# wfus/Fully-Homomorphic-Image-Processing

Measured on AMD Instinct MI355X. Metric: encrypted 8x8 blocks/sec (homomorphic DCT+quant), higher is better.
Workload: dtype f64

## Files before the change

### fully-homomorphic-image-processing_amd/csrc/dct_fused.hip

```cpp
#include "internal.h"

#include <cstdlib>

#include "fp64_core.h"

#pragma clang fp contract(off)

namespace {
using namespace fp64;

template <int L, int LE> struct Shape {
    static constexpr int N = 1 << L, E = 1 << LE, TP = N >> LE, NP = (L + LE - 1) / LE, LDS_WORDS = N + (N >> LE);
};
__host__ __device__ constexpr int g_lo(int L, int LE, int p) { return (L - LE * p - LE) < 0 ? 0 : (L - LE * p - LE); }
__host__ __device__ constexpr int g_stages(int L, int LE, int p) { return (L - LE * p) > LE ? LE : (L - LE * p); }
template <int LO, int LE> __device__ __forceinline__ int g_index(int tid, int r) {
    return ((tid >> LO) << (LO + LE)) | (r << LO) | (tid & ((1 << LO) - 1));
}
template <int LO, int LE> __device__ __forceinline__ int g_pad(int j) { return j + ((j >> (LO + LE)) << LO); }

template <int L, int LE, int P> struct PassTw {
    static constexpr int LO = g_lo(L, LE, P), S = g_stages(L, LE, P), NTW = (1 << LE) - 1;
    static constexpr int rb(int u) { return (L - 1 - (LE * P + u)) - LO; }
    static constexpr int count(int u) { return 1 << (LE - 1 - rb(u)); }
// ... 22 lines not shown
            double t[KB * M], wm[KB * M];
#pragma unroll
            for (int kb = 0; kb < KB; kb++) {
                const int b = b0 + kb, r0 = ((b >> rb) << (rb + 1)) | (b & ((1 << rb) - 1)), r1 = r0 | (1 << rb);
                const double wv = w[T::offset(u) + (r0 >> (rb + 1))];
#pragma unroll
                for (int m = 0; m < M; m++) { t[kb * M + m] = x[m][r1]; wm[kb * M + m] = wv; }
            }
            mmv<KB * M>(t, wm, p, pinv);
#pragma unroll
            for (int kb = 0; kb < KB; kb++) {
                const int b = b0 + kb, r0 = ((b >> rb) << (rb + 1)) | (b & ((1 << rb) - 1)), r1 = r0 | (1 << rb);
#pragma unroll
                for (int m = 0; m < M; m++) {
                    const double X = x[m][r0];
                    x[m][r0] = X + t[kb * M + m];
                    x[m][r1] = X - t[kb * M + m];
                }
            }
        }
    }
}

template <int L, int LE, int P, int M>
__device__ __forceinline__ void inv_pass(double (&x)[M][1 << LE], const double (&w)[(1 << LE) - 1], double ninv, double p, double pinv) {
    using T = PassTw<L, LE, P>;
    constexpr int E = 1 << LE, KB = (LE == 3) ? 2 : 1;
#pragma unroll
    for (int u = T::S - 1; u >= 0; u--) {
        const int sigma = LE * P + u, rb = T::rb(u);
        if (sigma == 0) {
#pragma unroll
            for (int b = 0; b < E / 2; b++) {
                const int r0 = ((b >> rb) << (rb + 1)) | (b & ((1 << rb) - 1)), r1 = r0 | (1 << rb);
                const double wv = w[T::offset(u) + (r0 >> (rb + 1))];
                double t[2 * M], wm[2 * M];
#pragma unroll
                for (int m = 0; m < M; m++) {
                    const double X = x[m][r0], Y = x[m][r1];
                    t[m] = X + Y; wm[m] = ninv;
                    t[M + m] = X - Y; wm[M + m] = wv;
                }
                mmv<2 * M>(t, wm, p, pinv);
#pragma unroll
                for (int m = 0; m < M; m++) { x[m][r0] = t[m]; x[m][r1] = t[M + m]; }
            }
        } else {
#pragma unroll
            for (int b0 = 0; b0 < E / 2; b0 += KB) {
                double t[KB * M], wm[KB * M];
#pragma unroll
                for (int kb = 0; kb < KB; kb++) {
                    const int b = b0 + kb, r0 = ((b >> rb) << (rb + 1)) | (b & ((1 << rb) - 1)), r1 = r0 | (1 << rb);
                    const double wv = w[T::offset(u) + (r0 >> (rb + 1))];
#pragma unroll
                    for (int m = 0; m < M; m++) {
                        const double X = x[m][r0], Y = x[m][r1];
                        x[m][r0] = X + Y;
                        t[kb * M + m] = X - Y; wm[kb * M + m] = wv;
                    }
                }
                mmv<KB * M>(t, wm, p, pinv);
#pragma unroll
                for (int kb = 0; kb < KB; kb++) {
                    const int b = b0 + kb, r0 = ((b >> rb) << (rb + 1)) | (b & ((1 << rb) - 1)), r1 = r0 | (1 << rb);
#pragma unroll
                    for (int m = 0; m < M; m++) x[m][r1] = t[kb * M + m];
                }
            }
        }
    }
}

template <int L, int LE, int LO_FROM, int LO_TO, int M>
__device__ __forceinline__ void transpose(double (&x)[M][1 << LE], double *lds, int tid, int &phase) {
    constexpr int PL = imin(LO_FROM, LO_TO), E = 1 << LE;
    constexpr bool WAVE_LOCAL = (Shape<L, LE>::TP <= 64) || (LO_FROM <= 6 && LO_TO <= 6);
#pragma unroll
    for (int m = 0; m < M; m++) {
        double *buf = lds + (phase & 1) * Shape<L, LE>::LDS_WORDS;
        phase++;
#pragma unroll
        for (int r = 0; r < E; r++) buf[g_pad<PL, LE>(g_index<LO_FROM, LE>(tid, r))] = x[m][r];
        if constexpr (WAVE_LOCAL) {
            __builtin_amdgcn_fence(__ATOMIC_RELEASE, "wavefront");
            __builtin_amdgcn_wave_barrier();
            __builtin_amdgcn_fence(__ATOMIC_ACQUIRE, "wavefront");
        } else {
            __syncthreads();
        }
#pragma unroll
        for (int r = 0; r < E; r++) x[m][r] = buf[g_pad<PL, LE>(g_index<LO_TO, LE>(tid, r))];
    }
}

template <int L, int LE, int M, typename PRE, int P = 0>
__device__ __forceinline__ void ntt_fwd(double (&x)[M][1 << LE], double (&w)[(1 << LE) - 1], const double *__restrict__ tw, double p, double pinv,
                                        double *lds, int tid, int &phase, PRE pre) {
    if constexpr (P + 1 < Shape<L, LE>::NP) {
        double wn[(1 << LE) - 1];
        if (LE >= 4) load_tw<L, LE, P + 1>(wn, tw, tid);
        fwd_pass<L, LE, P, M>(x, w, p, pinv);
        if (LE < 4) load_tw<L, LE, P + 1>(wn, tw, tid);
        if constexpr (P + 2 == Shape<L, LE>::NP) pre();
        transpose<L, LE, g_lo(L, LE, P), g_lo(L, LE, P + 1), M>(x, lds, tid, phase);
        ntt_fwd<L, LE, M, PRE, P + 1>(x, wn, tw, p, pinv, lds, tid, phase, pre);
    } else {
        fwd_pass<L, LE, P, M>(x, w, p, pinv);
    }
}
template <int L, int LE, int M, bool BIG, int P = Shape<L, LE>::NP - 1>
__device__ __forceinline__ void ntt_inv(double (&x)[M][1 << LE], double (&w)[(1 << LE) - 1], const double *__restrict__ itw, double p, double pinv,
                                        double *lds, int tid, int &phase) {
    if constexpr (P > 0) {
        double wn[(1 << LE) - 1];
        if (LE >= 4) load_tw<L, LE, P - 1>(wn, itw, tid);
        inv_pass<L, LE, P, M>(x, w, 0.0, p, pinv);
        if (LE < 4) load_tw<L, LE, P - 1>(wn, itw, tid);
        if constexpr (BIG) {
#pragma unroll
            for (int m = 0; m < M; m++)
#pragma unroll
                for (int r = 0; r < (1 << LE); r++) x[m][r] = red(x[m][r], p, pinv);
        }
        transpose<L, LE, g_lo(L, LE, P), g_lo(L, LE, P - 1), M>(x, lds, tid, phase);
        ntt_inv<L, LE, M, BIG, P - 1>(x, wn, itw, p, pinv, lds, tid, phase);
    } else {
        inv_pass<L, LE, P, M>(x, w, itw[0], p, pinv);
    }
}

constexpr double PACK_BIAS = 6755399441055744.0;
template <int E, int TP>
__device__ __forceinline__ void store_packed(char *__restrict__ ob, u32 vo, u32 so, const double (&x)[E]) {
    static_assert(E == 8, "packed layout is defined for 8 values per thread");
    u32 lo[8], hi[8];
#pragma unroll
    for (int r = 0; r < 8; r++) {
        const double t = x[r] + PACK_BIAS;
        lo[r] = (u32)__double2loint(t);
        hi[r] = (u32)__double2hiint(t);
    }
#pragma unroll
    for (int q = 0; q < 4; q++) *(u64 *)(ob + (size_t)(so + q * TP * 8) + vo) = (u64)lo[2 * q] | ((u64)lo[2 * q + 1] << 32);
    u32 h[2];
#pragma unroll
    for (int g = 0; g < 2; g++) {
        const u32 p01 = __builtin_amdgcn_perm(hi[4 * g + 1], hi[4 * g + 0], 0x0c0c0400u);
        const u32 p23 = __builtin_amdgcn_perm(hi[4 * g + 3], hi[4 * g + 2], 0x0c0c0400u);
        h[g] = __builtin_amdgcn_perm(p23, p01, 0x05040100u);
    }
// ... 113 lines not shown
        }
    }
}

__host__ __device__ constexpr int occ_waves(int tp, int lds_words) {
    return ((2 * lds_words * 16 <= 160 * 1024) ? 2 : 1) * tp / 256 < 1 ? 1 : ((2 * lds_words * 16 <= 160 * 1024) ? 2 : 1) * tp / 256;
}
template <int L, int LE> struct Occ { static constexpr int W = occ_waves(Shape<L, LE>::TP, Shape<L, LE>::LDS_WORDS); };

template <int L, int LE, bool BIG, bool PACK, bool LDSC>
__global__ __launch_bounds__((Shape<L, LE>::TP), (Occ<L, LE>::W)) void k_dct_rows(const u64 *__restrict__ in, double *__restrict__ mid,
                                                                  const double *__restrict__ consts, const double *__restrict__ tw_all,
                                                                  const Modulus *__restrict__ mods, u32 k) {
    __shared__ double lds[2 * Shape<L, LE>::LDS_WORDS];
    const Work wk = decode(blockIdx.x, k);
    const double p = (double)mods[wk.prime].q, pinv = 1.0 / p;
    const double *tw = tw_all + (size_t)wk.prime * Shape<L, LE>::N;
    if (wk.half) rows_body<L, LE, BIG, 1, PACK, LDSC>(in, mid, consts, tw, wk, p, pinv, k, lds);
    else rows_body<L, LE, BIG, 0, PACK, LDSC>(in, mid, consts, tw, wk, p, pinv, k, lds);
}

template <int L, int LE, bool BIG, int HALF, bool PACK>
__device__ __forceinline__ void cols_body(const double *__restrict__ mid, u64 *__restrict__ out, const double *__restrict__ consts,
                                          const double *__restrict__ itw, const Work &wk, double p, double pinv, u32 k, double *lds) {
    using SH = Shape<L, LE>;
    constexpr int N = SH::N, TP = SH::TP, E = SH::E, NC = HalfC<HALF>::NC, FIRST = HalfC<HALF>::FIRST;
    constexpr int LASTP = SH::NP - 1;
    const int tid = threadIdx.x;
    const size_t poly_words = (size_t)k * N, ct_words = 2 * poly_words;
    const size_t base = ((size_t)wk.blk * 64 + wk.line) * ct_words + (size_t)wk.poly * poly_words + (size_t)wk.prime * N;
    const size_t cstride = (size_t)k * N;
    const gwin_t win_mid = gwin(mid + base), win_out = gwin(out + base);
    const gwin_t win_c = gwin(consts + (size_t)FIRST * cstride + (size_t)wk.prime * N);
    const gwin_t win_s = gwin(consts + (size_t)(12 + 8 * HALF + wk.line) * cstride + (size_t)wk.prime * N);
    const u32 vo = (u32)tid * 8u, rsb = (u32)(ct_words * 64), csb = (u32)(cstride * 8);
    const double pbias = p + 4503599627370496.0;
    double cn[9], sn[4];
    auto fetch = [&](int r) {
#pragma unroll
        for (int i = 0; i < NC; i++) cn[i] = gld_f64(win_c, vo, (u32)i * csb + r * TP * 8);
#pragma unroll
        for (int m = 0; m < 4; m++) sn[m] = gld_f64(win_s, vo, (u32)(16 * m) * csb + r * TP * 8);
    };
    double wl[E - 1];
    if constexpr (!PACK) {
        fetch(0);
        load_tw<L, LE, LASTP>(wl, itw, tid);
    }
    double x[4][E];
    if constexpr (PACK) {
// ... 25 lines not shown
            for (int r = 0; r < E; r++) {
                const double A = gld_f64(win_mid, vo, (u32)m * rsb + r * TP * 8), B = gld_f64(win_mid, vo, (u32)(7 - m) * rsb + r * TP * 8);
                x[m][r] = HALF ? A - B : A + B;
            }
        }
    }
    if constexpr (PACK) load_tw<L, LE, LASTP>(wl, itw, tid);
#pragma unroll
    for (int r = 0; r < E; r++) {
        double c[9], sc[4];
        if (PACK) fetch(r);
#pragma unroll
        for (int i = 0; i < NC; i++) c[i] = cn[i];
#pragma unroll
        for (int m = 0; m < 4; m++) sc[m] = sn[m];
        if (!PACK && r + 1 < E) fetch(r + 1);
        line_half<HALF>(x[0][r], x[1][r], x[2][r], x[3][r], c, p, pinv);
        double y[4] = {x[0][r], x[1][r], x[2][r], x[3][r]};
        mmv<4>(y, sc, p, pinv);
#pragma unroll
        for (int m = 0; m < 4; m++) x[m][r] = y[m];
    }
    int phase = 0;
    ntt_inv<L, LE, 4, BIG>(x, wl, itw, p, pinv, lds, tid, phase);
#pragma unroll
    for (int m = 0; m < 4; m++) {
#pragma unroll
        for (int r = 0; r < E; r++) gst_u64(win_out, vo, (u32)(2 * m + HALF) * rsb + r * TP * 8, f64_to_residue(x[m][r], pbias));
    }
}

template <int L, int LE, bool BIG, bool PACK>
__global__ __launch_bounds__((Shape<L, LE>::TP), (Occ<L, LE>::W)) void k_dct_cols(const double *__restrict__ mid, u64 *__restrict__ out,
                                                                  const double *__restrict__ consts, const double *__restrict__ itw_all,
                                                                  const Modulus *__restrict__ mods, u32 k) {
    __shared__ double lds[2 * Shape<L, LE>::LDS_WORDS];
    const Work wk = decode(blockIdx.x, k);
    const double p = (double)mods[wk.prime].q, pinv = 1.0 / p;
    const double *itw = itw_all + (size_t)wk.prime * Shape<L, LE>::N;
    if (wk.half) cols_body<L, LE, BIG, 1, PACK>(mid, out, consts, itw, wk, p, pinv, k, lds);
    else cols_body<L, LE, BIG, 0, PACK>(mid, out, consts, itw, wk, p, pinv, k, lds);
}

template <int L, int LE>
__global__ __launch_bounds__((Shape<L, LE>::TP), (Occ<L, LE>::W)) void k_dct_one_launch(const u64 *__restrict__ in, double *__restrict__ mid, u64 *__restrict__ out,
                                                                        const double *__restrict__ consts, const double *__restrict__ tw_all,
                                                                        const double *__restrict__ itw_all, const Modulus *__restrict__ mods, u32 k,
                                                                        u32 n_blocks, u32 dist, u32 *__restrict__ arrived, u32 *__restrict__ err) {
    __shared__ double lds[2 * Shape<L, LE>::LDS_WORDS];
    const u32 xcd = blockIdx.x & 7, seq = blockIdx.x >> 3, chunk = seq >> 5, r = seq & 31;
    const bool is_row = r < 16;
    const long j = is_row ? (long)chunk : (long)chunk - (long)(dist & 0xffffu);
    const u32 n_units = n_blocks * 2 * k;
    if (j < 0) return;
    const u64 g = (u64)j * 8 + xcd;
    if (g >= n_units) return;
    Work wk;
    wk.prime = (u32)(g / (n_blocks * 2));
    const u32 rem = (u32)(g - (u64)wk.prime * n_blocks * 2);
    wk.blk = rem >> 1;
    wk.poly = rem & 1;
    wk.line = (r & 15) >> 1;
    wk.half = r & 1;
    const double p = (double)mods[wk.prime].q, pinv = 1.0 / p;
    if (is_row) {
        const double *tw = tw_all + (size_t)wk.prime * Shape<L, LE>::N;
        if (wk.half) rows_body<L, LE, false, 1, true, true>(in, mid, consts, tw, wk, p, pinv, k, lds);
        else rows_body<L, LE, false, 0, true, true>(in, mid, consts, tw, wk, p, pinv, k, lds);
        if (dist & 0x10000u) return;
        __syncthreads();
        if (threadIdx.x == 0) {
            __threadfence();
            atomicAdd(arrived + g, 1u);
        }
    } else {
        if (!(dist & 0x10000u) && threadIdx.x == 0) {
            u32 spins = 0;
            while (__hip_atomic_load(arrived + g, __ATOMIC_RELAXED, __HIP_MEMORY_SCOPE_AGENT) < 16u) {
                __builtin_amdgcn_s_sleep(8);
                if (++spins > (1u << 24)) { atomicExch(err, 1u); break; }
            }
            __threadfence();
        }
        __syncthreads();
        const double *itw = itw_all + (size_t)wk.prime * Shape<L, LE>::N;
        if (wk.half) cols_body<L, LE, false, 1, true>(mid, out, consts, itw, wk, p, pinv, k, lds);
        else cols_body<L, LE, false, 0, true>(mid, out, consts, itw, wk, p, pinv, k, lds);
    }
}

__global__ void k_consts_to_f64(const ulonglong2 *__restrict__ in, double *__restrict__ out, const Modulus *__restrict__ mods, u32 k, u32 n, u32 le, u32 total) {
    const u32 i = blockIdx.x * blockDim.x + threadIdx.x;
    if (i >= total) return;
    const u32 pos = i % n, rowbase = i - pos;
    const u32 tp = n >> le, r = pos / tp, t = pos % tp;
    const u32 j = (t << le) + r;
    const u32 src = (j & 15) * (n >> 4) + (j >> 4);
    const u64 q = mods[(i / n) % k].q;
    const u64 w = in[rowbase + src].x;
    out[i] = w > q / 2 ? -(double)(q - w) : (double)w;
}

template <int L, int LE>
__global__ __launch_bounds__((Shape<L, LE>::TP), (Occ<L, LE>::W)) void k_rgb2ycc_f64(u64 *__restrict__ R, u64 *__restrict__ G, u64 *__restrict__ Bc,
                                                                     const double *__restrict__ consts, const double *__restrict__ tw_all,
                                                                     const double *__restrict__ itw_all, const Modulus *__restrict__ mods,
                                                                     const u64 *__restrict__ yoff, u32 yoff_len, u32 k, u32 group, u64 gstride) {
    using SH = Shape<L, LE>;
    constexpr int N = SH::N, TP = SH::TP, E = SH::E, LASTP = SH::NP - 1;
    __shared__ double lds[2 * SH::LDS_WORDS];
    const int tid = threadIdx.x;
    const u32 per_prime = gridDim.x / k;
    const u32 prime = blockIdx.x / per_prime;
    const u32 pp = blockIdx.x - prime * per_prime;
    const u32 poly = pp & 1, pix = pp >> 1;
    const u64 q = mods[prime].q;
    const double p = (double)q, pinv = 1.0 / p;
    const double *tw = tw_all + (size_t)prime * N, *itw = itw_all + (size_t)prime * N;
    const size_t pix_off = group ? (size_t)(pix / group) * gstride + (size_t)(pix % group) * 2 * k * N : (size_t)pix * 2 * k * N;
    const size_t off = pix_off + ((size_t)poly * k + prime) * N + tid;
    double w0[E - 1];
    load_tw<L, LE, 0>(w0, tw, tid);
// ... 112 lines not shown
            dst[r * TP] = f64_to_u52(v);
        }
    }
}

}


static u32 dct_shape_le(const fhe_ctx *c) {
    if (c->opt.dct_le != 3) return 4;
    if (c->logn == 12 && c->max_prime_bits <= 40) return 3;
    if (c->logn == 13 || c->logn == 11) return 3;
    return 4;
}

bool fhe_dct_f64_supported(const fhe_ctx *c) {
    return c && c->qb.d_tw_f64 && c->max_prime_bits <= 47 && (c->logn >= 10 && c->logn <= 13);
}

int fhe_dct_f64_make_consts(const fhe_ctx *c, fhe_dct_plan *plan, hipStream_t st) {
    const u32 total = DCT_NCONST * c->k * c->n;
    HIP_TRY(hipMalloc(&plan->d_consts_f64, sizeof(double) * total));
    const u32 le = dct_shape_le(c);
    k_consts_to_f64<<<(total + 255) / 256, 256, 0, st>>>(plan->d_consts, plan->d_consts_f64, c->qb.d_mod, c->k, c->n, le, total);
    KERNEL_CHECK();
    return FHE_OK;
}



template <int L, int LE>
static void launch_pair(const fhe_ctx *c, const fhe_dct_plan *plan, const u64 *in, u64 *out, double *mid, unsigned grid, bool big, hipStream_t st, int which) {
    constexpr int TP = Shape<L, LE>::TP;
    if constexpr (LE == 4) {
        if (big) {
            if (which & 1) k_dct_rows<L, LE, true, false, false><<<grid, TP, 0, st>>>(in, mid, plan->d_consts_f64, c->qb.d_tw_f64, c->qb.d_mod, c->k);
            if (which & 2) k_dct_cols<L, LE, true, false><<<grid, TP, 0, st>>>(mid, out, plan->d_consts_f64, c->qb.d_itw_f64, c->qb.d_mod, c->k);
            return;
        }
    }
    if constexpr (LE == 3) {
        if (big) {
            if (which & 1) k_dct_rows<L, LE, true, false, false><<<grid, TP, 0, st>>>(in, mid, plan->d_consts_f64, c->qb.d_tw_f64, c->qb.d_mod, c->k);
            if (which & 2) k_dct_cols<L, LE, true, false><<<grid, TP, 0, st>>>(mid, out, plan->d_consts_f64, c->qb.d_itw_f64, c->qb.d_mod, c->k);
            return;
        }
        if (c->max_prime_bits <= 37 && c->opt.dct_pack) {
            if (which & 1) {
                if (c->opt.dct_ldsc) k_dct_rows<L, LE, false, true, true><<<grid, TP, 0, st>>>(in, mid, plan->d_consts_f64, c->qb.d_tw_f64, c->qb.d_mod, c->k);
                else k_dct_rows<L, LE, false, true, false><<<grid, TP, 0, st>>>(in, mid, plan->d_consts_f64, c->qb.d_tw_f64, c->qb.d_mod, c->k);
            }
            if (which & 2) k_dct_cols<L, LE, false, true><<<grid, TP, 0, st>>>(mid, out, plan->d_consts_f64, c->qb.d_itw_f64, c->qb.d_mod, c->k);
            return;
        }
    }
    {
        if (which & 1) k_dct_rows<L, LE, false, false, false><<<grid, TP, 0, st>>>(in, mid, plan->d_consts_f64, c->qb.d_tw_f64, c->qb.d_mod, c->k);
        if (which & 2) k_dct_cols<L, LE, false, false><<<grid, TP, 0, st>>>(mid, out, plan->d_consts_f64, c->qb.d_itw_f64, c->qb.d_mod, c->k);
    }
}

int fhe_dct_f64_launch(const fhe_ctx *c, const fhe_dct_plan *plan, const u64 *in, u64 *out, u64 n_blocks, double *mid, hipStream_t st, int which) {
    const u64 items = n_blocks * 8 * 2 * c->k;
    const u64 grid = items * 2;
    if (grid > 0x7fffffffULL) return fail(FHE_ERR_PARAM, "too many blocks for one launch");
    if ((u64)c->k * c->n >= (1ULL << 21)) return fail(FHE_ERR_PARAM, "fused FP64 path: a block of ciphertexts exceeds the 2 GiB addressing window");
    const bool big = c->max_prime_bits > 40;
    if (c->opt.dct_one_launch && which == 3 && c->logn == 12 && dct_shape_le(c) == 3 && c->max_prime_bits <= 37 && c->opt.dct_pack && c->d_arrived) {
        const u64 n_units = n_blocks * 2 * c->k;
        if (n_units > c->arrived_cap) return fail(FHE_ERR_PARAM, "one-launch experiment: wave too large for the arrival counters");
        HIP_TRY(hipMemsetAsync(c->d_arrived, 0, (n_units + 1) * sizeof(u32), st));
        const u32 dist = c->opt.dct_one_launch;
        const u64 chunks = (n_units + 7) / 8 + (dist & 0xffffu);
        k_dct_one_launch<12, 3><<<(unsigned)(chunks * 32 * 8), Shape<12, 3>::TP, 0, st>>>(in, mid, out, plan->d_consts_f64, c->qb.d_tw_f64, c->qb.d_itw_f64, c->qb.d_mod,
                                                                                       c->k, (u32)n_blocks, dist, c->d_arrived + 1, c->d_arrived);
        KERNEL_CHECK();
        u32 timed_out = 0;
        HIP_TRY(hipMemcpyAsync(&timed_out, c->d_arrived, sizeof(u32), hipMemcpyDeviceToHost, st));
        HIP_TRY(hipStreamSynchronize(st));
        if (timed_out) return fail(FHE_ERR_HIP, "one-launch experiment: a column workgroup timed out waiting for its row transforms; the output is incomplete");
        return FHE_OK;
    }
    switch (c->logn) {
        case 10: launch_pair<10, 4>(c, plan, in, out, mid, (unsigned)grid, big, st, which); break;
        case 11: launch_pair<11, 3>(c, plan, in, out, mid, (unsigned)grid, big, st, which); break;
        case 12: if (dct_shape_le(c) == 3) launch_pair<12, 3>(c, plan, in, out, mid, (unsigned)grid, false, st, which); else launch_pair<12, 4>(c, plan, in, out, mid, (unsigned)grid, big, st, which); break;
        case 13: if (dct_shape_le(c) == 3) launch_pair<13, 3>(c, plan, in, out, mid, (unsigned)grid, big, st, which); else launch_pair<13, 4>(c, plan, in, out, mid, (unsigned)grid, big, st, which); break;
        default: return fail(FHE_ERR_PARAM, "fused FP64 path supports n in {1024, 2048, 4096, 8192}");
    }
    KERNEL_CHECK();
    return FHE_OK;
}

bool fhe_rgb_f64_supported(const fhe_ctx *c) {
    return fhe_dct_f64_supported(c) && c->logn == 12 && c->max_prime_bits <= 40;
}

int fhe_rgb_f64_make_consts(const fhe_ctx *c, const ulonglong2 *d_c, double **out, hipStream_t st) {
    const u32 total = 9 * c->k * c->n;
    HIP_TRY(hipMalloc(out, sizeof(double) * total));
    k_consts_to_f64<<<(total + 255) / 256, 256, 0, st>>>(d_c, *out, c->qb.d_mod, c->k, c->n, 3, total);
    KERNEL_CHECK();
    return FHE_OK;
}

int fhe_rgb_f64_launch(const fhe_ctx *c, u64 *r, u64 *g, u64 *b, u64 count, const double *consts, const u64 *yoff, u32 yoff_len, hipStream_t st, u32 group, u64 gstride) {
    const u64 grid = count * 2 * c->k;
    if (grid > 0x7fffffffULL) return fail(FHE_ERR_PARAM, "too many pixels for one launch");
    k_rgb2ycc_f64<12, 3><<<(unsigned)grid, Shape<12, 3>::TP, 0, st>>>(r, g, b, consts, c->qb.d_tw_f64, c->qb.d_itw_f64, c->qb.d_mod, yoff, yoff_len, c->k, group, gstride);
    KERNEL_CHECK();
    return FHE_OK;
}

int fhe_poly_f64_launch(int mode, const fhe_ctx *c, const u64 *in, u64 *out, u64 n_polys, const ulonglong2 *plain, hipStream_t st) {
    const u64 grid2 = (n_polys / 2) * c->k, grid1 = n_polys * c->k;
    if (grid1 > 0x7fffffffULL) return fail(FHE_ERR_PARAM, "too many polynomials for one launch");
    constexpr int TP = Shape<12, 3>::TP;
#define LAUNCH_POLY(M, GRID)                                                                                                          \
    switch (mode) {                                                                                                                   \
        case 0: k_poly_f64<12, 3, M, 0><<<(unsigned)(GRID), TP, 0, st>>>(in, out, plain, c->qb.d_tw_f64, c->qb.d_itw_f64, c->qb.d_mod, c->k); break; \
        case 1: k_poly_f64<12, 3, M, 1><<<(unsigned)(GRID), TP, 0, st>>>(in, out, plain, c->qb.d_tw_f64, c->qb.d_itw_f64, c->qb.d_mod, c->k); break; \
        default: k_poly_f64<12, 3, M, 2><<<(unsigned)(GRID), TP, 0, st>>>(in, out, plain, c->qb.d_tw_f64, c->qb.d_itw_f64, c->qb.d_mod, c->k); break; \
    }
    if (n_polys % 2 == 0) { LAUNCH_POLY(2, grid2) } else { LAUNCH_POLY(1, grid1) }
// ... 135 lines not shown
__global__ __launch_bounds__((Shape<L, LE>::TP), (Occ<L, LE>::W)) void k_idct_cols(const double *__restrict__ mid, u64 *__restrict__ out,
                                                                   const double *__restrict__ consts, const double *__restrict__ itw_all,
                                                                   const Modulus *__restrict__ mods, u32 k) {
    __shared__ double lds[2 * Shape<L, LE>::LDS_WORDS];
    const Work wk = decode(blockIdx.x, k);
    const double p = (double)mods[wk.prime].q, pinv = 1.0 / p;
    const double *itw = itw_all + (size_t)wk.prime * Shape<L, LE>::N;
    if (wk.half) icols_body<L, LE, BIG, 1>(mid, out, consts, itw, wk, p, pinv, k, lds);
    else icols_body<L, LE, BIG, 0>(mid, out, consts, itw, wk, p, pinv, k, lds);
}

template <int L, int LE>
void launch_ipair(const fhe_ctx *c, const double *consts, const u64 *in, u64 *out, double *mid, unsigned grid, bool big, hipStream_t st) {
    constexpr int TP = Shape<L, LE>::TP;
    k_idct_rows<L, LE><<<grid, TP, 0, st>>>(in, mid, consts, c->qb.d_tw_f64, c->qb.d_mod, c->k);
    if (big) k_idct_cols<L, LE, true><<<grid, TP, 0, st>>>(mid, out, consts, c->qb.d_itw_f64, c->qb.d_mod, c->k);
    else k_idct_cols<L, LE, false><<<grid, TP, 0, st>>>(mid, out, consts, c->qb.d_itw_f64, c->qb.d_mod, c->k);
}
}

int fhe_idct_f64_make_consts(const fhe_ctx *c, const ulonglong2 *d_consts, double **out, hipStream_t st) {
    const u32 total = DCT_NCONST * c->k * c->n;
    HIP_TRY(hipMalloc(out, sizeof(double) * total));
    k_consts_to_f64<<<(total + 255) / 256, 256, 0, st>>>(d_consts, *out, c->qb.d_mod, c->k, c->n, dct_shape_le(c), total);
    KERNEL_CHECK();
    return FHE_OK;
}

int fhe_idct_f64_launch(const fhe_ctx *c, const double *consts, const u64 *in, u64 *out, u64 n_blocks, double *mid, hipStream_t st) {
    const u64 grid = n_blocks * 8 * 2 * c->k * 2;
    if (grid > 0x7fffffffULL) return fail(FHE_ERR_PARAM, "too many blocks for one launch");
    const bool big = c->max_prime_bits > 40;
    switch (c->logn) {
        case 10: launch_ipair<10, 4>(c, consts, in, out, mid, (unsigned)grid, big, st); break;
        case 11: launch_ipair<11, 3>(c, consts, in, out, mid, (unsigned)grid, big, st); break;
        case 12: if (dct_shape_le(c) == 3) launch_ipair<12, 3>(c, consts, in, out, mid, (unsigned)grid, big, st); else launch_ipair<12, 4>(c, consts, in, out, mid, (unsigned)grid, big, st); break;
        case 13: if (dct_shape_le(c) == 3) launch_ipair<13, 3>(c, consts, in, out, mid, (unsigned)grid, big, st); else launch_ipair<13, 4>(c, consts, in, out, mid, (unsigned)grid, big, st); break;
        default: return fail(FHE_ERR_PARAM, "fused FP64 path supports n in {1024, 2048, 4096, 8192}");
    }
    KERNEL_CHECK();
    return FHE_OK;
}
```

### fully-homomorphic-image-processing_amd/csrc/fhe_hip.hip

```cpp
#include "internal.h"

#include <cmath>
#include <cstdarg>
#include <cstdio>
#include <cstdlib>
#include <cstring>
#include <algorithm>
#include <condition_variable>
#include <mutex>
#include <string>
#include <vector>

#include "host_math.h"

static thread_local std::string g_err;
int fhe_fail(int code, const char *fmt, ...) {
    char buf[512];
    va_list ap;
    va_start(ap, fmt);
    vsnprintf(buf, sizeof buf, fmt, ap);
    va_end(ap);
    g_err = buf;
    return code;
}

extern "C" const char *fhe_last_error(void) { return g_err.c_str(); }
extern "C" uint32_t fhe_abi_version(void) { return FHE_ABI_VERSION; }

int fhe_build_base(BaseTables &B, const std::vector<u64> &primes, u32 n, u32 logn, bool want_f64) {
    using namespace hostmath;
    const size_t cnt = primes.size();
    B.primes = primes;
    std::vector<ulonglong2> tw(cnt * n), itw(cnt * n);
    B.h_mod.resize(cnt);
    for (size_t i = 0; i < cnt; ++i) {
        const u64 q = primes[i];
        const u64 psi = primitive_2n_root(q, n);
        if (!psi) return fail(FHE_ERR_PARAM, "no primitive 2n-th root modulo %llu", (unsigned long long)q);
        const u64 ipsi = invmod(psi, q), ninv = invmod(n % q, q);
        u64 p = 1, ip = 1;
        for (u32 j = 0; j < n; ++j) {
            const u32 r = bit_reverse(j, (int)logn);
            tw[i * n + r] = make_ulonglong2(p, shoup(p, q));
            itw[i * n + r] = make_ulonglong2(ip, shoup(ip, q));
            p = mulmod(p, psi, q);
            ip = mulmod(ip, ipsi, q);
        }
        itw[i * n + 0] = make_ulonglong2(ninv, shoup(ninv, q));
        const u64 w1 = mulmod(itw[i * n + 1].x, ninv, q);
        itw[i * n + 1] = make_ulonglong2(w1, shoup(w1, q));
        Modulus m;
        m.q = q;
        const int b = bit_length(q);
        m.mu = (u64)((((u128)1) << (2 * b)) / q);
        m.s1 = (u32)(b - 1);
        m.s2 = (u32)(b + 1);
        B.h_mod[i] = m;
    }
    HIP_TRY(hipMalloc(&B.d_tw, sizeof(ulonglong2) * cnt * n));
    HIP_TRY(hipMalloc(&B.d_itw, sizeof(ulonglong2) * cnt * n));
    HIP_TRY(hipMalloc(&B.d_mod, sizeof(Modulus) * cnt));
    HIP_TRY(hipMemcpy(B.d_tw, tw.data(), sizeof(ulonglong2) * cnt * n, hipMemcpyHostToDevice));
    HIP_TRY(hipMemcpy(B.d_itw, itw.data(), sizeof(ulonglong2) * cnt * n, hipMemcpyHostToDevice));
    HIP_TRY(hipMemcpy(B.d_mod, B.h_mod.data(), sizeof(Modulus) * cnt, hipMemcpyHostToDevice));
    bool a_all = true, b_all = true;
    std::vector<PmMod> pm(cnt);
    for (size_t i = 0; i < cnt; ++i) {
        const u64 q = primes[i];
        const int b = bit_length(q);
        if (b < 34 || b > 58) { a_all = b_all = false; break; }
        const u64 delta = (1ULL << b) - q;
// ... 30 lines not shown
            auto p3 = [logn](u32 idx) -> u32 {
                if (idx < 2) return idx;
                int sigma = 0;
                while ((2u << sigma) <= idx) sigma++;
                const int LE = 3, P = sigma / LE, lo = ((int)logn - LE * P - LE) < 0 ? 0 : ((int)logn - LE * P - LE), rb = ((int)logn - 1 - sigma) - lo;
                const u32 off = idx - (1u << sigma), cnt_i = 1u << (LE - 1 - rb), th = off / cnt_i, i = off % cnt_i;
                return (1u << sigma) + i * ((1u << sigma) / cnt_i) + th;
            };
            for (size_t i = 0; i < cnt; ++i) {
                const u64 q = primes[i];
                for (u32 j = 0; j < n; ++j) {
                    const u32 jp = p3(j);
                    twp[i * n + jp] = make_ulonglong2(tw[i * n + j].x, (u64)(((u128)tw[i * n + j].x << 31) % q));
                    itwp[i * n + jp] = make_ulonglong2(itw[i * n + j].x, (u64)(((u128)itw[i * n + j].x << 31) % q));
                }
            }
            HIP_TRY(hipMalloc(&B.d_tw_pm3, sizeof(ulonglong2) * cnt * n));
            HIP_TRY(hipMalloc(&B.d_itw_pm3, sizeof(ulonglong2) * cnt * n));
            HIP_TRY(hipMemcpy(B.d_tw_pm3, twp.data(), sizeof(ulonglong2) * cnt * n, hipMemcpyHostToDevice));
            HIP_TRY(hipMemcpy(B.d_itw_pm3, itwp.data(), sizeof(ulonglong2) * cnt * n, hipMemcpyHostToDevice));
        }
    }
    if (want_f64) {
        std::vector<double> twd(cnt * n), itwd(cnt * n);
        for (size_t i = 0; i < cnt; ++i) {
            const u64 q = primes[i];
            auto centred = [q](u64 w) { return w > q / 2 ? -(double)(q - w) : (double)w; };
            for (u32 j = 0; j < n; ++j) {
                twd[i * n + j] = centred(tw[i * n + j].x);
                itwd[i * n + j] = centred(itw[i * n + j].x);
            }
        }
        HIP_TRY(hipMalloc(&B.d_tw_f64, sizeof(double) * cnt * n));
        HIP_TRY(hipMalloc(&B.d_itw_f64, sizeof(double) * cnt * n));
        HIP_TRY(hipMemcpy(B.d_tw_f64, twd.data(), sizeof(double) * cnt * n, hipMemcpyHostToDevice));
        HIP_TRY(hipMemcpy(B.d_itw_f64, itwd.data(), sizeof(double) * cnt * n, hipMemcpyHostToDevice));
    }
    return FHE_OK;
}
void fhe_free_base(BaseTables &B) {
    if (B.d_tw) (void)hipFree(B.d_tw);
    if (B.d_itw) (void)hipFree(B.d_itw);
    if (B.d_mod) (void)hipFree(B.d_mod);
    if (B.d_tw_f64) (void)hipFree(B.d_tw_f64);
    if (B.d_itw_f64) (void)hipFree(B.d_itw_f64);
    if (B.d_tw_pm) (void)hipFree(B.d_tw_pm);
    if (B.d_itw_pm) (void)hipFree(B.d_itw_pm);
    if (B.d_pm) (void)hipFree(B.d_pm);
    if (B.d_tw_pm3) (void)hipFree(B.d_tw_pm3);
    if (B.d_itw_pm3) (void)hipFree(B.d_itw_pm3);
    B.d_tw_pm = B.d_itw_pm = B.d_tw_pm3 = B.d_itw_pm3 = nullptr;
    B.d_pm = nullptr;
    B.pm_class = 0;
    B.d_tw_f64 = B.d_itw_f64 = nullptr;
    B.d_tw = B.d_itw = nullptr;
    B.d_mod = nullptr;
}

static bool env_on(const char *name) { const char *e = getenv(name); return e && *e && !(e[0] == '0' && !e[1]); }

extern "C" int fhe_default_coeff_modulus(uint32_t n, int preset, uint64_t *q_out) {
    static const u64 s3_4096[] = {0xffffee001ULL, 0xffffc4001ULL, 0x1ffffe0001ULL};
    static const u64 s3_8192[] = {0x7fffffd8001ULL, 0x7fffffc8001ULL, 0xfffffffc001ULL, 0xffffff6c001ULL, 0xfffffebc001ULL};
    static const u64 s23_2048[] = {0x3fffffff000001ULL};
    static const u64 s23_4096[] = {0x7fffffff380001ULL, 0x3fffffff000001ULL};
    static const u64 s23_8192[] = {0x7fffffff380001ULL, 0x7ffffffef00001ULL, 0x3fffffff000001ULL, 0x3ffffffef40001ULL};
    static const u64 s23_16384[] = {0x7fffffff380001ULL, 0x7ffffffef00001ULL, 0x7ffffffeac0001ULL, 0x7ffffffe700001ULL, 0x7ffffffe600001ULL, 0x7ffffffe4c0001ULL,
                                    0x3fffffff000001ULL, 0x3ffffffef40001ULL};
    const u64 *src = nullptr;
    int cnt = 0;
#define PICK(a) do { src = a; cnt = (int)(sizeof(a) / sizeof(a[0])); } while (0)
    if (preset == 0) {
        if (n == 4096) PICK(s3_4096);
        else if (n == 8192) PICK(s3_8192);
        else if (n == 2048 || n == 1024) PICK(s23_2048);
        else if (n == 16384) PICK(s23_16384);
    } else if (preset == 1) {
        if (n == 2048 || n == 1024) PICK(s23_2048);
// ... 1533 lines not shown
```

### fully-homomorphic-image-processing_amd/csrc/fp64_core.h

```cpp
#pragma once
#include "internal.h"

#pragma clang fp contract(off)

namespace fp64 {

__device__ __forceinline__ double mm(double y, double w, double p, double pinv) {
    const double h = y * w;
    const double l = __builtin_fma(y, w, -h);
    const double q = __builtin_rint(h * pinv);
    return __builtin_fma(-q, p, h) + l;
}
__device__ __forceinline__ double red(double x, double p, double pinv) {
    return __builtin_fma(-__builtin_rint(x * pinv), p, x);
}
template <int K>
__device__ __forceinline__ void mmv(double (&y)[K], const double (&w)[K], double p, double pinv) {
    double h[K], l[K], q[K];
#pragma unroll
    for (int i = 0; i < K; i++) h[i] = y[i] * w[i];
#pragma unroll
    for (int i = 0; i < K; i++) q[i] = h[i] * pinv;
#pragma unroll
    for (int i = 0; i < K; i++) l[i] = __builtin_fma(y[i], w[i], -h[i]);
#pragma unroll
    for (int i = 0; i < K; i++) q[i] = __builtin_rint(q[i]);
#pragma unroll
    for (int i = 0; i < K; i++) h[i] = __builtin_fma(-q[i], p, h[i]);
#pragma unroll
    for (int i = 0; i < K; i++) y[i] = h[i] + l[i];
}

__device__ __forceinline__ double u52_to_f64(u64 v) { return __longlong_as_double((long long)(v | 0x4330000000000000ULL)) - 4503599627370496.0; }
__device__ __forceinline__ u64 f64_to_u52(double v) { return (u64)__double_as_longlong(v + 4503599627370496.0) & 0x000FFFFFFFFFFFFFULL; }
__device__ __forceinline__ double u52_biased(u64 v) { return __longlong_as_double((long long)(v | 0x4330000000000000ULL)); }
__device__ __forceinline__ u64 f64_to_residue(double v, double pbias) {
    return (u64)__double_as_longlong(v + (v < 0.0 ? pbias : 4503599627370496.0)) & 0x000FFFFFFFFFFFFFULL;
}

typedef u32 u32x2 __attribute__((ext_vector_type(2)));
typedef __amdgpu_buffer_rsrc_t gwin_t;
__device__ __forceinline__ gwin_t gwin(const void *base) {
    return __builtin_amdgcn_make_buffer_rsrc(const_cast<void *>(base), 0, -1, 0x00020000 );
}
__device__ __forceinline__ u64 gld_u64(gwin_t w, u32 voff, u32 soff) { return __builtin_bit_cast(u64, __builtin_amdgcn_raw_buffer_load_b64(w, voff, soff, 0)); }
__device__ __forceinline__ double gld_f64(gwin_t w, u32 voff, u32 soff) { return __builtin_bit_cast(double, __builtin_amdgcn_raw_buffer_load_b64(w, voff, soff, 0)); }
__device__ __forceinline__ void gst_u64(gwin_t w, u32 voff, u32 soff, u64 v) { __builtin_amdgcn_raw_buffer_store_b64(__builtin_bit_cast(u32x2, v), w, voff, soff, 0); }
__device__ __forceinline__ void gst_f64(gwin_t w, u32 voff, u32 soff, double v) { __builtin_amdgcn_raw_buffer_store_b64(__builtin_bit_cast(u32x2, v), w, voff, soff, 0); }

template <int HALF>
__device__ __forceinline__ void line_half(double &x0, double &x1, double &x2, double &x3, const double (&c)[9], double p, double pinv) {
    if constexpr (HALF == 0) {
        const double tmp10 = x0 + x3, tmp13 = x0 - x3, tmp11 = x1 + x2, tmp12 = x1 - x2;
        double y[3] = {tmp12 + tmp13, tmp13, tmp12};
        const double w[3] = {c[0], c[1], c[2]};
        mmv<3>(y, w, p, pinv);
        x0 = tmp10 + tmp11;
        x2 = tmp10 - tmp11;
        x1 = y[0] + y[1];
        x3 = y[0] + y[2];
// ... 35 lines not shown
```

### fully-homomorphic-image-processing_amd/csrc/internal.h

```cpp
#pragma once
#include "../../include/fhe_hip.h"

#include <hip/hip_runtime.h>

#include <mutex>
#include <string>
#include <vector>

#include "modarith.h"
#include "ntt_core.h"

int fhe_fail(int code, const char *fmt, ...) __attribute__((format(printf, 2, 3)));
#define fail fhe_fail
#define HIP_TRY(expr)                                                                             \
    do {                                                                                          \
        hipError_t e_ = (expr);                                                                   \
        if (e_ != hipSuccess) return fail(FHE_ERR_HIP, "%s: %s", #expr, hipGetErrorString(e_));   \
    } while (0)
#define KERNEL_CHECK()                                                                            \
    do {                                                                                          \
        hipError_t e_ = hipGetLastError();                                                        \
        if (e_ != hipSuccess) return fail(FHE_ERR_HIP, "kernel launch: %s", hipGetErrorString(e_)); \
    } while (0)

struct BaseTables {
    std::vector<u64> primes;
    ulonglong2 *d_tw = nullptr, *d_itw = nullptr;
    Modulus *d_mod = nullptr;
    std::vector<Modulus> h_mod;
    double *d_tw_f64 = nullptr, *d_itw_f64 = nullptr;
    ulonglong2 *d_tw_pm = nullptr, *d_itw_pm = nullptr;
    ulonglong2 *d_tw_pm3 = nullptr, *d_itw_pm3 = nullptr;
    PmMod *d_pm = nullptr;
    int pm_class = 0;
    RnsBase dev() const { return RnsBase{d_tw, d_itw, d_mod, (u32)primes.size(), d_tw_pm, d_itw_pm, d_pm}; }
};

struct FheOptions {
    bool force_u64 = false;
    bool dct_pipeline = false;
    u64 dct_wave_blocks = 256;
    int dct_le = 3;
    bool dct_pack = true;
    bool dct_ldsc = true;
    bool dct_u64_fused = true;
    u32 dct_one_launch = 0;
    bool ntt_nolazy = false;
    bool ntt_single = false;
    bool ntt_nopm = false;
    bool behz_aux61 = false;
    bool behz_chunk3 = false;
    bool behz_tensor_canon = false;
    bool behz_tensor_single = false;
// ... 115 lines not shown
```

Measured before the change: 87070.

## Fold inverse-NTT n^-1 scaling into DCT constants and skip final-stage sum reduction

The inverse NTT's final stage no longer multiplies the sum half by n^-1. That factor is instead pre-multiplied into the DCT column constants (consts index ≥ 12) when they are converted to f64, and the last stage uses the raw first twiddle from a new per-prime table. This removes a modular multiply per sum output in the last inverse butterfly stage. Where needed, the unreduced sums are reduced with a cheap floor-based residue at store time (packed, non-big path) or an explicit red. The change relies on bounds proven via static_assert and touches constant-generation layout, so correctness depends on the folded constants matching every consumer.

```diff
diff --git a/fully-homomorphic-image-processing_amd/csrc/dct_fused.hip b/fully-homomorphic-image-processing_amd/csrc/dct_fused.hip
--- a/fully-homomorphic-image-processing_amd/csrc/dct_fused.hip
+++ b/fully-homomorphic-image-processing_amd/csrc/dct_fused.hip
@@ -68,14 +68,14 @@
     }
 }
 
-template <int L, int LE, int P, int M>
-__device__ __forceinline__ void inv_pass(double (&x)[M][1 << LE], const double (&w)[(1 << LE) - 1], double ninv, double p, double pinv) {
+template <int L, int LE, int P, int M, bool NINV_FOLDED = false, bool RED_SUMS = false>
+__device__ __forceinline__ void inv_pass(double (&x)[M][1 << LE], const double (&w)[(1 << LE) - 1], double last, double p, double pinv) {
     using T = PassTw<L, LE, P>;
     constexpr int E = 1 << LE, KB = (LE == 3) ? 2 : 1;
 #pragma unroll
     for (int u = T::S - 1; u >= 0; u--) {
         const int sigma = LE * P + u, rb = T::rb(u);
-        if (sigma == 0) {
+        if (sigma == 0 && !NINV_FOLDED) {
 #pragma unroll
             for (int b = 0; b < E / 2; b++) {
                 const int r0 = ((b >> rb) << (rb + 1)) | (b & ((1 << rb) - 1)), r1 = r0 | (1 << rb);
@@ -84,7 +84,7 @@
 #pragma unroll
                 for (int m = 0; m < M; m++) {
                     const double X = x[m][r0], Y = x[m][r1];
-                    t[m] = X + Y; wm[m] = ninv;
+                    t[m] = X + Y; wm[m] = last;
                     t[M + m] = X - Y; wm[M + m] = wv;
                 }
                 mmv<2 * M>(t, wm, p, pinv);
@@ -98,7 +98,7 @@
 #pragma unroll
                 for (int kb = 0; kb < KB; kb++) {
                     const int b = b0 + kb, r0 = ((b >> rb) << (rb + 1)) | (b & ((1 << rb) - 1)), r1 = r0 | (1 << rb);
-                    const double wv = w[T::offset(u) + (r0 >> (rb + 1))];
+                    const double wv = (sigma == 0) ? last : w[T::offset(u) + (r0 >> (rb + 1))];
 #pragma unroll
                     for (int m = 0; m < M; m++) {
                         const double X = x[m][r0], Y = x[m][r1];
@@ -112,6 +112,10 @@
                     const int b = b0 + kb, r0 = ((b >> rb) << (rb + 1)) | (b & ((1 << rb) - 1)), r1 = r0 | (1 << rb);
 #pragma unroll
                     for (int m = 0; m < M; m++) x[m][r1] = t[kb * M + m];
+                    if (sigma == 0 && RED_SUMS) {
+#pragma unroll
+                        for (int m = 0; m < M; m++) x[m][r0] = red(x[m][r0], p, pinv);
+                    }
                 }
             }
         }
@@ -155,9 +159,9 @@
         fwd_pass<L, LE, P, M>(x, w, p, pinv);
     }
 }
-template <int L, int LE, int M, bool BIG, int P = Shape<L, LE>::NP - 1>
+template <int L, int LE, int M, bool BIG, bool NINV_FOLDED = false, bool RED_SUMS = false, int P = Shape<L, LE>::NP - 1>
 __device__ __forceinline__ void ntt_inv(double (&x)[M][1 << LE], double (&w)[(1 << LE) - 1], const double *__restrict__ itw, double p, double pinv,
-                                        double *lds, int tid, int &phase) {
+                                        double *lds, int tid, int &phase, double wlast = 0.0) {
     if constexpr (P > 0) {
         double wn[(1 << LE) - 1];
         if (LE >= 4) load_tw<L, LE, P - 1>(wn, itw, tid);
@@ -170,9 +174,10 @@
                 for (int r = 0; r < (1 << LE); r++) x[m][r] = red(x[m][r], p, pinv);
         }
         transpose<L, LE, g_lo(L, LE, P), g_lo(L, LE, P - 1), M>(x, lds, tid, phase);
-        ntt_inv<L, LE, M, BIG, P - 1>(x, wn, itw, p, pinv, lds, tid, phase);
+        ntt_inv<L, LE, M, BIG, NINV_FOLDED, RED_SUMS, P - 1>(x, wn, itw, p, pinv, lds, tid, phase, wlast);
     } else {
-        inv_pass<L, LE, P, M>(x, w, itw[0], p, pinv);
+        static_assert(PassTw<L, LE, 0>::rb(0) == LE - 1, "last inverse stage must pair slot r with slot r + E / 2");
+        inv_pass<L, LE, P, M, NINV_FOLDED, RED_SUMS>(x, w, NINV_FOLDED ? wlast : itw[0], p, pinv);
     }
 }
 
@@ -332,10 +337,13 @@
 
 template <int L, int LE, bool BIG, int HALF, bool PACK>
 __device__ __forceinline__ void cols_body(const double *__restrict__ mid, u64 *__restrict__ out, const double *__restrict__ consts,
-                                          const double *__restrict__ itw, const Work &wk, double p, double pinv, u32 k, double *lds) {
+                                          const double *__restrict__ itw, double wlast, const Work &wk, double p, double pinv, u32 k, double *lds) {
     using SH = Shape<L, LE>;
     constexpr int N = SH::N, TP = SH::TP, E = SH::E, NC = HalfC<HALF>::NC, FIRST = HalfC<HALF>::FIRST;
     constexpr int LASTP = SH::NP - 1;
+    constexpr bool FLOOR_RES = PACK && !BIG && L <= 13;
+    static_assert(!FLOOR_RES || (1 << L) * 6 / 10 < FLOOR_RESIDUE_MAX_RATIO, "sum outputs exceed the range f64_floor_residue is proven for");
+    constexpr bool RED_AT_STORE = !FLOOR_RES && L == 10, RED_IN_STAGE = !FLOOR_RES && !RED_AT_STORE;
     const int tid = threadIdx.x;
     const size_t poly_words = (size_t)k * N, ct_words = 2 * poly_words;
     const size_t base = ((size_t)wk.blk * 64 + wk.line) * ct_words + (size_t)wk.poly * poly_words + (size_t)wk.prime * N;
@@ -407,30 +415,37 @@
         for (int m = 0; m < 4; m++) x[m][r] = y[m];
     }
     int phase = 0;
-    ntt_inv<L, LE, 4, BIG>(x, wl, itw, p, pinv, lds, tid, phase);
+    ntt_inv<L, LE, 4, BIG, true, RED_IN_STAGE>(x, wl, itw, p, pinv, lds, tid, phase, wlast);
 #pragma unroll
     for (int m = 0; m < 4; m++) {
 #pragma unroll
-        for (int r = 0; r < E; r++) gst_u64(win_out, vo, (u32)(2 * m + HALF) * rsb + r * TP * 8, f64_to_residue(x[m][r], pbias));
+        for (int r = 0; r < E; r++) {
+            u64 o;
+            if (FLOOR_RES && r < E / 2) o = f64_floor_residue(x[m][r], p, pinv);
+            else if (RED_AT_STORE && r < E / 2) o = f64_to_residue(red(x[m][r], p, pinv), pbias);
+            else o = f64_to_residue(x[m][r], pbias);
+            gst_u64(win_out, vo, (u32)(2 * m + HALF) * rsb + r * TP * 8, o);
+        }
     }
 }
 
 template <int L, int LE, bool BIG, bool PACK>
 __global__ __launch_bounds__((Shape<L, LE>::TP), (Occ<L, LE>::W)) void k_dct_cols(const double *__restrict__ mid, u64 *__restrict__ out,
                                                                   const double *__restrict__ consts, const double *__restrict__ itw_all,
-                                                                  const Modulus *__restrict__ mods, u32 k) {
+                                                                  const double *__restrict__ itw1_all, const Modulus *__restrict__ mods, u32 k) {
     __shared__ double lds[2 * Shape<L, LE>::LDS_WORDS];
     const Work wk = decode(blockIdx.x, k);
     const double p = (double)mods[wk.prime].q, pinv = 1.0 / p;
     const double *itw = itw_all + (size_t)wk.prime * Shape<L, LE>::N;
-    if (wk.half) cols_body<L, LE, BIG, 1, PACK>(mid, out, consts, itw, wk, p, pinv, k, lds);
-    else cols_body<L, LE, BIG, 0, PACK>(mid, out, consts, itw, wk, p, pinv, k, lds);
+    const double wlast = itw1_all[wk.prime];
+    if (wk.half) cols_body<L, LE, BIG, 1, PACK>(mid, out, consts, itw, wlast, wk, p, pinv, k, lds);
+    else cols_body<L, LE, BIG, 0, PACK>(mid, out, consts, itw, wlast, wk, p, pinv, k, lds);
 }
 
 template <int L, int LE>
 __global__ __launch_bounds__((Shape<L, LE>::TP), (Occ<L, LE>::W)) void k_dct_one_launch(const u64 *__restrict__ in, double *__restrict__ mid, u64 *__restrict__ out,
                                                                         const double *__restrict__ consts, const double *__restrict__ tw_all,
-                                                                        const double *__restrict__ itw_all, const Modulus *__restrict__ mods, u32 k,
+                                                                        const double *__restrict__ itw_all, const double *__restrict__ itw1_all, const Modulus *__restrict__ mods, u32 k,
                                                                         u32 n_blocks, u32 dist, u32 *__restrict__ arrived, u32 *__restrict__ err) {
     __shared__ double lds[2 * Shape<L, LE>::LDS_WORDS];
     const u32 xcd = blockIdx.x & 7, seq = blockIdx.x >> 3, chunk = seq >> 5, r = seq & 31;
@@ -469,20 +484,27 @@
         }
         __syncthreads();
         const double *itw = itw_all + (size_t)wk.prime * Shape<L, LE>::N;
-        if (wk.half) cols_body<L, LE, false, 1, true>(mid, out, consts, itw, wk, p, pinv, k, lds);
-        else cols_body<L, LE, false, 0, true>(mid, out, consts, itw, wk, p, pinv, k, lds);
-    }
-}
-
-__global__ void k_consts_to_f64(const ulonglong2 *__restrict__ in, double *__restrict__ out, const Modulus *__restrict__ mods, u32 k, u32 n, u32 le, u32 total) {
+        const double wlast = itw1_all[wk.prime];
+        if (wk.half) cols_body<L, LE, false, 1, true>(mid, out, consts, itw, wlast, wk, p, pinv, k, lds);
+        else cols_body<L, LE, false, 0, true>(mid, out, consts, itw, wlast, wk, p, pinv, k, lds);
+    }
+}
+
+__global__ void k_consts_to_f64(const ulonglong2 *__restrict__ in, double *__restrict__ out, const Modulus *__restrict__ mods, u32 k, u32 n, u32 le, u32 total,
+                                const ulonglong2 *__restrict__ itw, u32 fold_first) {
     const u32 i = blockIdx.x * blockDim.x + threadIdx.x;
     if (i >= total) return;
     const u32 pos = i % n, rowbase = i - pos;
     const u32 tp = n >> le, r = pos / tp, t = pos % tp;
     const u32 j = (t << le) + r;
     const u32 src = (j & 15) * (n >> 4) + (j >> 4);
-    const u64 q = mods[(i / n) % k].q;
-    const u64 w = in[rowbase + src].x;
+    const u32 prime = (i / n) % k;
+    const u64 q = mods[prime].q;
+    u64 w = in[rowbase + src].x;
+    if (i / (k * n) >= fold_first) {
+        const ulonglong2 ninv = itw[(size_t)prime * n];
+        w = mul_shoup(w, ninv.x, ninv.y, q);
+    }
     out[i] = w > q / 2 ? -(double)(q - w) : (double)w;
 }
 
@@ -641,7 +663,7 @@
     const u32 total = DCT_NCONST * c->k * c->n;
     HIP_TRY(hipMalloc(&plan->d_consts_f64, sizeof(double) * total));
     const u32 le = dct_shape_le(c);
-    k_consts_to_f64<<<(total + 255) / 256, 256, 0, st>>>(plan->d_consts, plan->d_consts_f64, c->qb.d_mod, c->k, c->n, le, total);
+    k_consts_to_f64<<<(total + 255) / 256, 256, 0, st>>>(plan->d_consts, plan->d_consts_f64, c->qb.d_mod, c->k, c->n, le, total, c->qb.d_itw, 12);
     KERNEL_CHECK();
     return FHE_OK;
 }
@@ -654,14 +676,14 @@
     if constexpr (LE == 4) {
         if (big) {
             if (which & 1) k_dct_rows<L, LE, true, false, false><<<grid, TP, 0, st>>>(in, mid, plan->d_consts_f64, c->qb.d_tw_f64, c->qb.d_mod, c->k);
-            if (which & 2) k_dct_cols<L, LE, true, false><<<grid, TP, 0, st>>>(mid, out, plan->d_consts_f64, c->qb.d_itw_f64, c->qb.d_mod, c->k);
+            if (which & 2) k_dct_cols<L, LE, true, false><<<grid, TP, 0, st>>>(mid, out, plan->d_consts_f64, c->qb.d_itw_f64, c->qb.d_itw1_f64, c->qb.d_mod, c->k);
             return;
         }
     }
     if constexpr (LE == 3) {
         if (big) {
             if (which & 1) k_dct_rows<L, LE, true, false, false><<<grid, TP, 0, st>>>(in, mid, plan->d_consts_f64, c->qb.d_tw_f64, c->qb.d_mod, c->k);
-            if (which & 2) k_dct_cols<L, LE, true, false><<<grid, TP, 0, st>>>(mid, out, plan->d_consts_f64, c->qb.d_itw_f64, c->qb.d_mod, c->k);
+            if (which & 2) k_dct_cols<L, LE, true, false><<<grid, TP, 0, st>>>(mid, out, plan->d_consts_f64, c->qb.d_itw_f64, c->qb.d_itw1_f64, c->qb.d_mod, c->k);
             return;
         }
         if (c->max_prime_bits <= 37 && c->opt.dct_pack) {
@@ -669,13 +691,13 @@
                 if (c->opt.dct_ldsc) k_dct_rows<L, LE, false, true, true><<<grid, TP, 0, st>>>(in, mid, plan->d_consts_f64, c->qb.d_tw_f64, c->qb.d_mod, c->k);
                 else k_dct_rows<L, LE, false, true, false><<<grid, TP, 0, st>>>(in, mid, plan->d_consts_f64, c->qb.d_tw_f64, c->qb.d_mod, c->k);
             }
-            if (which & 2) k_dct_cols<L, LE, false, true><<<grid, TP, 0, st>>>(mid, out, plan->d_consts_f64, c->qb.d_itw_f64, c->qb.d_mod, c->k);
+            if (which & 2) k_dct_cols<L, LE, false, true><<<grid, TP, 0, st>>>(mid, out, plan->d_consts_f64, c->qb.d_itw_f64, c->qb.d_itw1_f64, c->qb.d_mod, c->k);
             return;
         }
     }
     {
         if (which & 1) k_dct_rows<L, LE, false, false, false><<<grid, TP, 0, st>>>(in, mid, plan->d_consts_f64, c->qb.d_tw_f64, c->qb.d_mod, c->k);
-        if (which & 2) k_dct_cols<L, LE, false, false><<<grid, TP, 0, st>>>(mid, out, plan->d_consts_f64, c->qb.d_itw_f64, c->qb.d_mod, c->k);
+        if (which & 2) k_dct_cols<L, LE, false, false><<<grid, TP, 0, st>>>(mid, out, plan->d_consts_f64, c->qb.d_itw_f64, c->qb.d_itw1_f64, c->qb.d_mod, c->k);
     }
 }
 
@@ -691,7 +713,7 @@
         HIP_TRY(hipMemsetAsync(c->d_arrived, 0, (n_units + 1) * sizeof(u32), st));
         const u32 dist = c->opt.dct_one_launch;
         const u64 chunks = (n_units + 7) / 8 + (dist & 0xffffu);
-        k_dct_one_launch<12, 3><<<(unsigned)(chunks * 32 * 8), Shape<12, 3>::TP, 0, st>>>(in, mid, out, plan->d_consts_f64, c->qb.d_tw_f64, c->qb.d_itw_f64, c->qb.d_mod,
+        k_dct_one_launch<12, 3><<<(unsigned)(chunks * 32 * 8), Shape<12, 3>::TP, 0, st>>>(in, mid, out, plan->d_consts_f64, c->qb.d_tw_f64, c->qb.d_itw_f64, c->qb.d_itw1_f64, c->qb.d_mod,
                                                                                        c->k, (u32)n_blocks, dist, c->d_arrived + 1, c->d_arrived);
         KERNEL_CHECK();
         u32 timed_out = 0;
@@ -718,7 +740,7 @@
 int fhe_rgb_f64_make_consts(const fhe_ctx *c, const ulonglong2 *d_c, double **out, hipStream_t st) {
     const u32 total = 9 * c->k * c->n;
     HIP_TRY(hipMalloc(out, sizeof(double) * total));
-    k_consts_to_f64<<<(total + 255) / 256, 256, 0, st>>>(d_c, *out, c->qb.d_mod, c->k, c->n, 3, total);
+    k_consts_to_f64<<<(total + 255) / 256, 256, 0, st>>>(d_c, *out, c->qb.d_mod, c->k, c->n, 3, total, c->qb.d_itw, ~0u);
     KERNEL_CHECK();
     return FHE_OK;
 }
@@ -900,7 +922,7 @@
 int fhe_idct_f64_make_consts(const fhe_ctx *c, const ulonglong2 *d_consts, double **out, hipStream_t st) {
     const u32 total = DCT_NCONST * c->k * c->n;
     HIP_TRY(hipMalloc(out, sizeof(double) * total));
-    k_consts_to_f64<<<(total + 255) / 256, 256, 0, st>>>(d_consts, *out, c->qb.d_mod, c->k, c->n, dct_shape_le(c), total);
+    k_consts_to_f64<<<(total + 255) / 256, 256, 0, st>>>(d_consts, *out, c->qb.d_mod, c->k, c->n, dct_shape_le(c), total, c->qb.d_itw, ~0u);
     KERNEL_CHECK();
     return FHE_OK;
 }
diff --git a/fully-homomorphic-image-processing_amd/csrc/fhe_hip.hip b/fully-homomorphic-image-processing_amd/csrc/fhe_hip.hip
--- a/fully-homomorphic-image-processing_amd/csrc/fhe_hip.hip
+++ b/fully-homomorphic-image-processing_amd/csrc/fhe_hip.hip
@@ -32,6 +32,7 @@
     const size_t cnt = primes.size();
     B.primes = primes;
     std::vector<ulonglong2> tw(cnt * n), itw(cnt * n);
+    std::vector<u64> itw1_plain(cnt);
     B.h_mod.resize(cnt);
     for (size_t i = 0; i < cnt; ++i) {
         const u64 q = primes[i];
@@ -47,6 +48,7 @@
             ip = mulmod(ip, ipsi, q);
         }
         itw[i * n + 0] = make_ulonglong2(ninv, shoup(ninv, q));
+        itw1_plain[i] = itw[i * n + 1].x;
         const u64 w1 = mulmod(itw[i * n + 1].x, ninv, q);
         itw[i * n + 1] = make_ulonglong2(w1, shoup(w1, q));
         Modulus m;
@@ -123,7 +125,7 @@
         }
     }
     if (want_f64) {
-        std::vector<double> twd(cnt * n), itwd(cnt * n);
+        std::vector<double> twd(cnt * n), itwd(cnt * n), itw1d(cnt);
         for (size_t i = 0; i < cnt; ++i) {
             const u64 q = primes[i];
             auto centred = [q](u64 w) { return w > q / 2 ? -(double)(q - w) : (double)w; };
@@ -131,11 +133,14 @@
                 twd[i * n + j] = centred(tw[i * n + j].x);
                 itwd[i * n + j] = centred(itw[i * n + j].x);
             }
+            itw1d[i] = centred(itw1_plain[i]);
         }
         HIP_TRY(hipMalloc(&B.d_tw_f64, sizeof(double) * cnt * n));
         HIP_TRY(hipMalloc(&B.d_itw_f64, sizeof(double) * cnt * n));
+        HIP_TRY(hipMalloc(&B.d_itw1_f64, sizeof(double) * cnt));
         HIP_TRY(hipMemcpy(B.d_tw_f64, twd.data(), sizeof(double) * cnt * n, hipMemcpyHostToDevice));
         HIP_TRY(hipMemcpy(B.d_itw_f64, itwd.data(), sizeof(double) * cnt * n, hipMemcpyHostToDevice));
+        HIP_TRY(hipMemcpy(B.d_itw1_f64, itw1d.data(), sizeof(double) * cnt, hipMemcpyHostToDevice));
     }
     return FHE_OK;
 }
@@ -145,6 +150,7 @@
     if (B.d_mod) (void)hipFree(B.d_mod);
     if (B.d_tw_f64) (void)hipFree(B.d_tw_f64);
     if (B.d_itw_f64) (void)hipFree(B.d_itw_f64);
+    if (B.d_itw1_f64) (void)hipFree(B.d_itw1_f64);
     if (B.d_tw_pm) (void)hipFree(B.d_tw_pm);
     if (B.d_itw_pm) (void)hipFree(B.d_itw_pm);
     if (B.d_pm) (void)hipFree(B.d_pm);
@@ -153,8 +159,8 @@
     B.d_tw_pm = B.d_itw_pm = B.d_tw_pm3 = B.d_itw_pm3 = nullptr;
     B.d_pm = nullptr;
     B.pm_class = 0;
-    B.d_tw_f64 = B.d_itw_f64 = nullptr;
-    B.d_tw = B.d_itw = nullptr;
+    B.d_tw_f64 = B.d_itw_f64 = B.d_itw1_f64 = nullptr;
+    B.d_tw =B.d_itw = nullptr;
     B.d_mod = nullptr;
 }
 
diff --git a/fully-homomorphic-image-processing_amd/csrc/fp64_core.h b/fully-homomorphic-image-processing_amd/csrc/fp64_core.h
--- a/fully-homomorphic-image-processing_amd/csrc/fp64_core.h
+++ b/fully-homomorphic-image-processing_amd/csrc/fp64_core.h
@@ -36,6 +36,13 @@
 __device__ __forceinline__ double u52_biased(u64 v) { return __longlong_as_double((long long)(v | 0x4330000000000000ULL)); }
 __device__ __forceinline__ u64 f64_to_residue(double v, double pbias) {
     return (u64)__double_as_longlong(v + (v < 0.0 ? pbias : 4503599627370496.0)) & 0x000FFFFFFFFFFFFFULL;
+}
+constexpr double FLOOR_RESIDUE_EPS = 0x1p-38;
+constexpr int FLOOR_RESIDUE_MAX_PRIME_BITS = 37, FLOOR_RESIDUE_MAX_RATIO = 4916;
+__device__ __forceinline__ u64 f64_floor_residue(double x, double p, double pinv) {
+    const double q = __builtin_floor(__builtin_fma(x, pinv, FLOOR_RESIDUE_EPS));
+    const double r = __builtin_fma(-q, p, x);
+    return (u64)__double_as_longlong(r + 4503599627370496.0) & 0x000FFFFFFFFFFFFFULL;
 }
 
 typedef u32 u32x2 __attribute__((ext_vector_type(2)));
diff --git a/fully-homomorphic-image-processing_amd/csrc/internal.h b/fully-homomorphic-image-processing_amd/csrc/internal.h
--- a/fully-homomorphic-image-processing_amd/csrc/internal.h
+++ b/fully-homomorphic-image-processing_amd/csrc/internal.h
@@ -29,6 +29,7 @@
     Modulus *d_mod = nullptr;
     std::vector<Modulus> h_mod;
     double *d_tw_f64 = nullptr, *d_itw_f64 = nullptr;
+    double *d_itw1_f64 = nullptr;
     ulonglong2 *d_tw_pm = nullptr, *d_itw_pm = nullptr;
     ulonglong2 *d_tw_pm3 = nullptr, *d_itw_pm3 = nullptr;
     PmMod *d_pm = nullptr;
```

After: 87470 (median of 4 runs). About the same (+0.5%).
